# CPOMUCL/GPSat

Measured on AMD Instinct MI355X. Metric: local-expert tiles/sec (fit+predict), higher is better.
Workload: dtype f32; 1 GPU; BASELINE.json configs[1]: synthetic tiles, RBF, 3D inputs, fp32; tiles_per_gpu=4096, pred_per_tile=500, dim=3, kernel=RBF, optimiser=lbfgs, max_iter=20, early_stopping=ftol/gtol defaults, failed_tiles=0, parallelism=tile-sharded x1, device=AMD Radeon Graphics (gfx950:sramecc+:xnack-)

## Files before the change

gpsat_amd/csrc/gpsat_capi.cpp:

```cpp
#include <hip/hip_runtime.h>
#include <algorithm>
#include <cmath>
#include <cstdio>
#include <cstdlib>
#include <cstring>
#include <limits>
#include <numeric>
#include <string>
#include <vector>

#include "gpsat_hip.h"
#include "gpsat_kernels.h"
#include "gpsat_plan.h"
#include "gpsat_cvfold.h"
#include "gpsat_select_plan.h"
#include "gpsat_bin_plan.h"

namespace {

thread_local std::string g_err;

int fail(int code, const std::string& msg) {
    g_err = msg;
    return code;
// ... 435 lines not shown
    HIP_TRY(hipMemsetAsync(h->pq.p, 0, head, h->stream));
    char* q = static_cast<char*>(h->pq.p);
    a.pq_ctl = reinterpret_cast<int*>(q);
    a.cu_busy = reinterpret_cast<int*>(q + 256);
    a.pq = reinterpret_cast<unsigned long long*>(q + 256 + 2048 * sizeof(int));
    a.pq_snap = reinterpret_cast<float*>(q + head);
    a.pq_stride = p.pq_stride; a.pq_slots = (int)slots;
    return GPSAT_OK;
}

struct LaunchReport {
    std::vector<int> team, coop;
    int pq_taken = -1, unfinished = 0;
    bool team_gave_up = false;
};

int queue_report(gpsat_handle* h, const gpsat::TilePlan& p, const gpsat::KernelArgs& a, LaunchReport& r) {
    if (p.team > 1) {
        r.team.resize((size_t)(p.grid / p.team) * 64);
        HIP_TRY(hipMemcpyAsync(r.team.data(), h->coop.p, r.team.size() * sizeof(int), hipMemcpyDeviceToHost, h->stream));
    }
    if (p.coop && dev_env("GPSAT_DEBUG_COOP_STATS")) {
        r.coop.resize((size_t)p.grid * 256);
        HIP_TRY(hipMemcpyAsync(r.coop.data(), h->coop.p, (size_t)p.grid * 1024, hipMemcpyDeviceToHost, h->stream));
    }
    if (a.pq_ctl && dev_env("GPSAT_DEBUG_DEFER_STATS"))
        HIP_TRY(hipMemcpyAsync(&r.pq_taken, a.pq_ctl, sizeof(int), hipMemcpyDeviceToHost, h->stream));
    if (p.seg_cost > 0) HIP_TRY(hipMemcpyAsync(&r.unfinished, a.ring_ctl + 32, sizeof(int), hipMemcpyDeviceToHost, h->stream));
    return GPSAT_OK;
}

void read_report(const gpsat::TilePlan& p, const gpsat::KernelArgs& a, LaunchReport& r) {
    const int grid = p.grid, T = a.T;
    if (!r.coop.empty()) {
        long long st[8] = {0};
        for (int g = 0; g < grid; ++g) for (int i = 0; i < 8; ++i) st[i] += r.coop[(size_t)g * 256 + 32 + GPSAT_PT_MAXNB + i];
        std::fprintf(stderr, "gpsat coop: grid %d T %d: cooperative evaluations %lld, helper phases %lld, helper groups (sweep) %lld, "
                             "flag waits given up %lld, owner waits given up %lld, pivot failures %lld, helper unwinds %lld\n",
                     grid, T, st[0], st[1], st[2], st[3], st[4], st[5], st[6]);
    }
    if (dev_env("GPSAT_DEBUG_DEFER_STATS"))
        std::fprintf(stderr, "gpsat defer: T %d: deferred predictions %d of %d snapshot slots\n", T,
                     r.pq_taken < 0 ? 0 : std::min(r.pq_taken, a.pq_slots), a.pq_slots);
    if (!r.team.empty() && dev_env("GPSAT_DEBUG_TEAM_STATS"))
        std::fprintf(stderr, "gpsat team 0 (size %d), factorisation, owner thread 0, s_memtime ticks: own work of (A) %d, (A) wait + barrier %d, (B) + barrier %d, "
                             "(C) + barrier %d\n", p.team, r.team[24], r.team[25], r.team[26], r.team[27]);
    for (size_t g = 0; g < r.team.size() / 64; ++g)
        if (r.team[g * 64 + 5]) r.team_gave_up = true;
}

struct DenseJob {
    const gpsat_batch* b;
    const gpsat_multistart* ms;
    const gpsat_cv* cv = nullptr;
    CvTables cv_tables;
    bool ms_on;
    BatchDims dims;
    const double* theta0;
    std::vector<double> theta0_clipped, starts_clipped;
    std::vector<int> order;
};

int run_tiles(gpsat_handle* h, const DenseJob& j, bool solo, bool unsliced, LaunchReport& r) {
    const gpsat_batch* b = j.b;
    const BatchDims& d = j.dims;
    const bool f64 = b->dtype == GPSAT_F64;
    gpsat::PlanInput in = {b->T, b->D, f64, b->obs_off, d.maxP, d.want_cov, d.sumP > 0, b->optimiser, b->max_iter,
                           h->num_cu, h->wg_per_cu, solo || j.cv, unsliced, read_dev_knobs()};
    gpsat::TilePlan p;
    if (!gpsat::plan_tiles(in, p)) return fail(GPSAT_EINVAL, "tile too large for LDS");
    Staged s;
    int rc;
    const size_t ws_bytes = (size_t)(p.grid / p.team) * p.ws_stride * (f64 ? sizeof(double) : sizeof(float));
    if ((rc = stage_batch(h, b, d, j.theta0, j.order, d.want_cov ? b->cov_off : nullptr, nullptr, ws_bytes, s))) return rc;
    gpsat::KernelArgs a;
    fill_common_args(a, b, s);
    a.NBmax = p.NBmax;
    a.ws = static_cast<float*>(h->ws.p); a.ws_stride = p.ws_stride;
    a.prof = nullptr;
    a.cov_off = d.want_cov ? s.i64 + 2 * (b->T + 1) : nullptr;
    a.f_cov = d.want_cov ? reinterpret_cast<float*>(s.cov) : nullptr;
    a.PCmax = p.PCcov;
    a.dump = nullptr; a.dump_stride = 0;
    if ((rc = setup_ring(h, p, j.order, a))) return rc;
    if ((rc = setup_coop_and_team(h, p, &b->T, a))) return rc;
    if (j.ms_on && (rc = setup_multistart(h, b, j.ms->n_starts, j.theta0, j.starts_clipped, a))) return rc;
    if ((rc = setup_deferred(h, p, a))) return rc;
    gpsat::CvArgs ca;
    if (j.cv) {
        if (!gpsat::builds[p.build].launch_cv) return fail(GPSAT_EINVAL, "held-out predictions: no kernel in this build");
        if ((rc = stage_cv(h, b, j.cv, d, j.cv_tables, ca))) return rc;
    }
#ifdef GPSAT_DUMP
    if (h->dump_dev && !f64) {
        const size_t need = ((size_t)p.NBmax * p.NBmax + p.NBmax) * 1024 + 2 * (size_t)p.NBmax * 32 + 16 + 8 * 1024;
        if (h->dump_stride < need) return fail(GPSAT_EINVAL, "dump stride too small: need " + std::to_string(need) + " floats per tile");
        a.dump = h->dump_dev; a.dump_stride = h->dump_stride;
    }
#endif
#ifdef GPSAT_PROFILE
    if ((rc = h->prof.reserve(sizeof(h->prof_host)))) return rc;
    HIP_TRY(hipMemsetAsync(h->prof.p, 0, sizeof(h->prof_host), h->stream));
    a.prof = static_cast<unsigned long long*>(h->prof.p);
#endif
    HIP_TRY(hipEventRecord(h->ev[1], h->stream));
    if (j.cv) HIP_TRY(gpsat::builds[p.build].launch_cv(b->D, a, ca, p.grid, p.smem, h->stream));
    else HIP_TRY(gpsat::builds[p.build].launch(b->D, a, p.grid, p.smem, h->stream));
    HIP_TRY(hipEventRecord(h->ev[2], h->stream));
    if ((rc = fetch_batch(h, b, d, s))) return rc;
    if (j.cv && (rc = fetch_cv(h, b, j.cv, d, ca))) return rc;
    if (j.ms_on && j.ms->f_start)
        HIP_TRY(hipMemcpyAsync(j.ms->f_start, a.ms_fout, (size_t)b->T * j.ms->n_starts * sizeof(double), hipMemcpyDeviceToHost, h->stream));
#ifdef GPSAT_PROFILE
    HIP_TRY(hipMemcpyAsync(h->prof_host, h->prof.p, sizeof(h->prof_host), hipMemcpyDeviceToHost, h->stream));
#endif
    if ((rc = queue_report(h, p, a, r))) return rc;
    HIP_TRY(hipEventRecord(h->ev[3], h->stream));
    HIP_TRY(hipStreamSynchronize(h->stream));
    read_report(p, a, r);
    return GPSAT_OK;
}

int fit_predict(gpsat_handle* h, const gpsat_batch* b, const gpsat_multistart* ms, const gpsat_cv* cv = nullptr) {
    if (!h || !b) return fail(GPSAT_EINVAL, "gpsat_fit_predict_batch: NULL handle or batch");
    if (b->T == 0) return GPSAT_OK;
    DenseJob j;
    j.b = b; j.ms = ms; j.cv = cv;
    int rc;
    if ((rc = check_batch(b, false, j.dims))) return rc;
    BatchDims& d = j.dims;
    d.want_cov = b->f_cov != nullptr;
    if (d.want_cov) {
        if (!b->cov_off) return fail(GPSAT_EINVAL, "f_cov given without cov_off");
        if (b->cov_off[0] != 0) return fail(GPSAT_EINVAL, "cov_off must start at 0");
        for (int t = 0; t < b->T; ++t) {
            const long long p = b->pred_off[t + 1] - b->pred_off[t];
            if (b->cov_off[t + 1] - b->cov_off[t] != p * p) return fail(GPSAT_EINVAL, "cov_off[t+1]-cov_off[t] must equal P_t^2");
            d.maxP = std::max(d.maxP, p);
        }
        d.sumC = b->cov_off[b->T];
    }
    if (d.maxN > gpsat_max_tile_obs(b->dtype, b->D))
        return fail(GPSAT_EINVAL, "tile too large for the LDS of a CU: at most " + std::to_string(gpsat_max_tile_obs(b->dtype, b->D)) +
                                      " observations per tile for this dtype and D (gpsat_max_tile_obs)");
    if ((rc = check_batch_data(b, d))) return rc;
    if (cv && (rc = check_cv(b, cv, d, j.cv_tables))) return rc;
    j.ms_on = ms && b->optimiser != GPSAT_OPT_NONE && b->max_iter > 0;
    if (ms && (rc = check_multistart(b, ms, j.ms_on, j.theta0_clipped, j.starts_clipped))) return rc;
    j.theta0 = j.ms_on ? j.theta0_clipped.data() : b->theta0;
    if ((rc = begin_call(h))) return rc;
    j.order.resize(b->T);
    std::iota(j.order.begin(), j.order.end(), 0);
    std::stable_sort(j.order.begin(), j.order.end(), [&](int a, int c) {
        return (b->obs_off[a + 1] - b->obs_off[a]) > (b->obs_off[c + 1] - b->obs_off[c]);
    });
    for (bool solo = false, unsliced = false;;) {
        LaunchReport r;
        if ((rc = run_tiles(h, j, solo, unsliced, r))) return rc;
        if (r.team_gave_up) {
            std::fprintf(stderr, "gpsat: a team barrier gave up; re-running the batch with one workgroup per tile\n");
            solo = true;
        } else if (r.unfinished != 0) {
            if (unsliced) return fail(GPSAT_EHIP, "tile queue ended with " + std::to_string(r.unfinished) + " unfinished tiles");
            std::fprintf(stderr, "gpsat: time-sliced tile queue ended with %d unfinished tiles; re-running the batch unsliced\n", r.unfinished);
            unsliced = true;
        } else {
// ... 663 lines not shown
```

gpsat_amd/csrc/gpsat_kernels.h:

```cpp
#ifndef GPSAT_KERNELS_H
#define GPSAT_KERNELS_H
#include <hip/hip_runtime.h>
#include <stddef.h>

#include "gpsat_select_types.h"

#define GPSAT_MAX_TILE_OBS 4096
#define GPSAT_PT_MAXNB 128
static_assert(32 * GPSAT_PT_MAXNB >= GPSAT_MAX_TILE_OBS, "fp32 sweep flags must cover the largest tile gpsat_max_tile_obs allows");

namespace gpsat {

constexpr int MS_WORDS = 16;

struct KernelArgs {
    int T, kernel, optimiser, max_iter, max_ls, NBmax;
    double ftol, gtol, adam_lr;
    double noise_rel;
    const long long* obs_off;
    const long long* pred_off;
    const double* theta0;
    const double* lo;
    const double* hi;
    const unsigned char* trainable;
    const float* X;
    const float* y;
    const float* Xs;
    double* theta;
    double* nll;
    double* grad;
    int* status;
    int* n_eval;
    int* n_iter;
    float* f_mean;
    float* f_var;
    float* y_var;
    const int* order;
    int* queue;
    float* ws;
    size_t ws_stride;
    unsigned long long* prof;
    const long long* cov_off;
    float* f_cov;
    int PCmax;
    unsigned long long* ring;
    int* ring_ctl;
    unsigned* state;
    int ring_mask, state_words, seg_cost;
    void* coop;
    int* coop_live;
    int team_size;
    void* team_ctl;
    int coop_min_nb;
    int coop_hdiv;
    int coop_force;
    float* dump;
    size_t dump_stride;
    unsigned long long* pq;
    int* pq_ctl;
    int* cu_busy;
    float* pq_snap;
    size_t pq_stride;
    int pq_slots;
    int ms_S = 0;
    const double* ms_starts = nullptr;
    double* ms_state = nullptr;
    double* ms_fout = nullptr;
};

struct CvArgs {
    const int* pair_off = nullptr;
    const int* pairs = nullptr;
    const int* fold_off = nullptr;
    const int* fold_ptr = nullptr;
    const int* fold_rows = nullptr;
    const int* fold_a = nullptr;
    const int* row_fold = nullptr;
    const int* row_pos = nullptr;
    double* mean = nullptr;
    double* f_var = nullptr;
    double* y_var = nullptr;
};
#define GPSAT_MAX_CV_FOLD 256

size_t shared_bytes(int D, int NBmax);
size_t shared_bytes_f64(int D, int NBmax);
size_t workspace_doubles_per_wg_f64(int NBmax, int PCcov);
int state_words_f64();
hipError_t launch_tiles_f64(int D, const KernelArgs& a, int grid, size_t smem, hipStream_t stream);
hipError_t launch_tiles_cv_f64(int D, const KernelArgs& a, const CvArgs& cv, int grid, size_t smem, hipStream_t stream);
size_t shared_bytes_f64_w4(int D, int NBmax);
size_t workspace_doubles_per_wg_f64_w4(int NBmax, int PCcov);
int state_words_f64_w4();
hipError_t launch_tiles_f64_w4(int D, const KernelArgs& a, int grid, size_t smem, hipStream_t stream);
hipError_t launch_tiles_cv_f64_w4(int D, const KernelArgs& a, const CvArgs& cv, int grid, size_t smem, hipStream_t stream);
size_t pq_floats_per_slot(int D, int NBmax);
size_t workspace_floats_per_wg(int NBmax, int PCcov);
hipError_t launch_tiles(int D, const KernelArgs& a, int grid, size_t smem, hipStream_t stream);
int state_words();
size_t shared_bytes_w8(int D, int NBmax);
size_t workspace_floats_per_wg_w8(int NBmax, int PCcov);
hipError_t launch_tiles_w8(int D, const KernelArgs& a, int grid, size_t smem, hipStream_t stream);
int state_words_w8();

struct SelectArgs : SelectCriteria {
    long long M;
    int C;
    int T;
    const double* pts;
    const double* refs;
    int n_chunks;
    long long chunk_rows;
    long long* counts;
    const long long* off;
    int* idx;
    const double* box;
    const int* eorder;
    int n_bounds;
    const double* bounds;
};

hipError_t launch_select(const SelectArgs& a, bool fill, hipStream_t stream);
hipError_t launch_select_boxes(long long M, int C, const double* pts, double* box, hipStream_t stream);
int select_sub_rows();

hipError_t select_bin_rows(long long M, int C, const double* pts, const BinSpec& b, unsigned* keys, unsigned* keys_out, int* rows,
                           int* perm, double* pts_perm, void* temp, size_t& temp_bytes, hipStream_t stream);
hipError_t select_unbin(int T, long long total, const unsigned* seg_off, const int* perm, int* idx, int* idx_out, void* temp,
                        size_t& temp_bytes, hipStream_t stream);

#ifndef GPSAT_BIN_COUNT
#define GPSAT_BIN_COUNT  1u
#define GPSAT_BIN_SUM    2u
#define GPSAT_BIN_MEAN   4u
#define GPSAT_BIN_STD    8u
#define GPSAT_BIN_MIN    16u
#define GPSAT_BIN_MAX    32u
#define GPSAT_BIN_MEDIAN 64u
#endif
struct BinArgs {
    long long R;
    int nx, ny;
    const double *x, *y, *v;
    const int* gid;
    const double *ex, *ey;
    double x_hi, y_hi;
    double inv_x, inv_y;
    unsigned long long sentinel;
    unsigned long long *keys, *keys_sorted;
    unsigned *rows, *perm;
// ... 78 lines not shown
```

gpsat_amd/csrc/gpsat_kernels.hip:

```cpp
#include <hip/hip_runtime.h>
#include <stdint.h>
#include "gpsat_kernels.h"
#include "gpsat_ring.h"

#ifdef GPSAT_PROFILE
#define PROF_BEGIN() unsigned long long prof_t_ = __builtin_amdgcn_s_memtime()
#define PROF_END(c_, slot_)                                                                  \
    do {                                                                                     \
        unsigned long long t1_ = __builtin_amdgcn_s_memtime();                               \
        if ((c_).lane == 0) (c_).prof[(c_).w * 16 + (slot_)] += t1_ - prof_t_;               \
        prof_t_ = t1_;                                                                       \
    } while (0)
#define TRACE(c_, code_, arg_)                                                                        \
    do {                                                                                              \
        if ((c_).trace && (c_).lane == 0 && shared_state()->tron) {                                   \
            const int i_ = shared_state()->tcnt[(c_).w]++;                                            \
            if (i_ < 1024) (c_).trace[(c_).w * 1024 + i_] = (__builtin_amdgcn_s_memtime() << 16) |    \
                                                           ((unsigned long long)((arg_) & 255) << 8) | (code_); \
        }                                                                                             \
    } while (0)
#else
#define PROF_BEGIN() do {} while (0)
#define PROF_END(c_, slot_) do {} while (0)
#define TRACE(c_, code_, arg_) do {} while (0)
// ... 168 lines not shown
__device__ __forceinline__ void wave_lds_sync() {
    asm volatile("" ::: "memory");
    __builtin_amdgcn_wave_barrier();
    asm volatile("" ::: "memory");
}

__device__ __forceinline__ int wave_pull(int* counter, int lane) {
    int v = 0;
    if (lane == 0) v = atomicAdd(counter, 1);
    return __builtin_amdgcn_readfirstlane(v);
}

template <int KERN>
struct KScale {
    static constexpr float c = (KERN == 0) ? 0.8493218002880191f : 1.0f;
    static constexpr float c2 = (KERN == 0) ? 0.7213475204444817f : 1.0f;
};

template <int KERN>
__device__ __forceinline__ void kfun(float r2, float& kf, float& gg) {
    if (KERN == 0) {
        kf = __builtin_amdgcn_exp2f(-r2);
        gg = kf;
    } else {
        float r = sqrtf(fmaxf(r2, 1e-36f));
        if (KERN == 1) {
            kf = __expf(-r);
            gg = kf / r;
        } else if (KERN == 2) {
            float s = 1.7320508075688772f * r;
            float e = __expf(-s);
            kf = (1.f + s) * e;
            gg = 3.f * e;
        } else {
            float s = 2.23606797749979f * r;
            float e = __expf(-s);
            kf = (1.f + s + s * s * (1.f / 3.f)) * e;
            gg = (5.f / 3.f) * (1.f + s) * e;
        }
    }
}

#define GPSAT_PT_FLAGS
#include "gpsat_opt.h"
#include "gpsat_coop.h"

constexpr int SHARED_FLOATS = (int)((sizeof(Shared) + 15) / 16) * 4;

__device__ __forceinline__ Shared* shared_state() { return reinterpret_cast<Shared*>(lds_f); }

struct Lay { int xs, xsc, y, z, alpha, Ad, LT, U01, Wh, tmp, piv, end; };

__host__ __device__ constexpr Lay lds_layout(int D, int NBmax) {
    const int NPmax = NBmax * 32;
    Lay L{};
    int off = SHARED_FLOATS;
    L.xs = off; off += D * NPmax;
    L.xsc = off; off += D * NPmax;
    L.y = off; off += NPmax;
    L.z = off; off += NPmax;
    L.alpha = off; off += NPmax;
    L.LT = off; off += 4 * BLK;
    L.U01 = off; off += 2 * BLK;
    L.Wh = off; off += 4 * BLK;
    L.Ad = off; off += 32 * 33 + 3;
    off = (off + 3) & ~3;
    L.tmp = off; off += 32;
    L.piv = off; off += 64;
    L.end = off;
    return L;
}
constexpr int LDS_SLACK_FLOATS = 3;

template <int D, int KN>
struct Ctx {
    Lay L;
    float* ws;
    int zb, dT0, vs0, cv0;
    int gp0;
    gCoopCtl* ctl;
    gfloat* zg;
    gfloat* ag;
    bool helper;
    int N, NB, Npad, P;
    int tid, lane, w, h, g;
    float sf2, sn2;
    unsigned long long* prof;
    unsigned long long* trace;
};

template <int D, int KERN>
__device__ __forceinline__ f32x16 kblock_t(const Ctx<D, KERN>& c, int bi, int bj) {
    const int q = 32 * bj + c.g;
    float xq[D];
#pragma unroll
    for (int d = 0; d < D; ++d) xq[d] = lds_f[c.L.xsc + d * c.Npad + q];
    f32x16 out;
    if (bi != bj && 32 * bi + 32 <= c.N && 32 * bj + 32 <= c.N) {
#pragma unroll
        for (int qq = 0; qq < 4; ++qq) {
            const int p0 = 32 * bi + 8 * qq + 4 * c.h;
            f32x2 r2[2];
#pragma unroll
            for (int d = 0; d < D; ++d) {
                const f32x4 xp = *reinterpret_cast<const f32x4*>(lds_f + c.L.xsc + d * c.Npad + p0);
                const f32x2 xb = {xq[d], xq[d]};
#pragma unroll
                for (int e = 0; e < 2; ++e) {
                    const f32x2 xa = {xp[2 * e], xp[2 * e + 1]};
                    const f32x2 df = xa - xb;
                    r2[e] = (d == 0) ? df * df : __builtin_elementwise_fma(df, df, r2[e]);
                }
            }
#pragma unroll
            for (int e = 0; e < 4; ++e) {
                float kf, gg;
                kfun<KERN>(r2[e >> 1][e & 1], kf, gg);
                out[4 * qq + e] = c.sf2 * kf;
            }
        }
        return out;
    }
#pragma unroll
    for (int qq = 0; qq < 4; ++qq) {
        const int p0 = 32 * bi + 8 * qq + 4 * c.h;
        float r2[4] = {0.f, 0.f, 0.f, 0.f};
#pragma unroll
        for (int d = 0; d < D; ++d) {
            f32x4 xp = *reinterpret_cast<const f32x4*>(lds_f + c.L.xsc + d * c.Npad + p0);
#pragma unroll
            for (int e = 0; e < 4; ++e) { float df = xp[e] - xq[d]; r2[e] = fmaf(df, df, r2[e]); }
        }
#pragma unroll
        for (int e = 0; e < 4; ++e) {
            const int p = p0 + e;
            float kf, gg;
            kfun<KERN>(r2[e], kf, gg);
            float v = c.sf2 * kf;
            const bool valid = (p < c.N) && (q < c.N);
            v = valid ? v : 0.f;
            if (p == q) v = (p < c.N) ? (v + c.sn2) : 1.f;
            out[4 * qq + e] = v;
        }
    }
    return out;
}

template <int D, int KN>
__device__ __forceinline__ f32x16 kblock(const Ctx<D, KN>& c, int bi, int bj) {
    return kblock_t<D, KN>(c, bi, bj);
}

template <int D, int KERN>
__device__ __forceinline__ f32x16 ksblock_t(const Ctx<D, KERN>& c, int bj, const float (&xq)[D], bool qvalid) {
    f32x16 out;
#pragma unroll
    for (int qq = 0; qq < 4; ++qq) {
        const int p0 = 32 * bj + 8 * qq + 4 * c.h;
        float r2[4] = {0.f, 0.f, 0.f, 0.f};
#pragma unroll
        for (int d = 0; d < D; ++d) {
            f32x4 xp = *reinterpret_cast<const f32x4*>(lds_f + c.L.xsc + d * c.Npad + p0);
#pragma unroll
            for (int e = 0; e < 4; ++e) { float df = xp[e] - xq[d]; r2[e] = fmaf(df, df, r2[e]); }
        }
#pragma unroll
// ... 307 lines not shown
        __builtin_amdgcn_s_sleep(2);
        if (++spins > (1 << 22)) {
            __hip_atomic_store(&sh->fail, 2, __ATOMIC_RELAXED, __HIP_MEMORY_SCOPE_WORKGROUP);
            return false;
        }
    }
    __builtin_amdgcn_fence(__ATOMIC_ACQUIRE, "workgroup");
    return true;
}

__device__ __forceinline__ bool pt_wait_lc(Shared* sh, gCoopCtl* ctl, const int* flag, int v) {
    int spins = 0;
    while (__hip_atomic_load(flag, RLX_WG) < v) {
        if (__hip_atomic_load(&sh->fail, RLX_WG)) return false;
        __builtin_amdgcn_s_sleep(2);
        ++spins;
        if (((spins & 63) == 0 && __hip_atomic_load(&ctl->fail, RLX_AGENT)) || spins > (1 << 22)) {
            __hip_atomic_store(&sh->fail, 2, RLX_WG);
            return false;
        }
    }
    __builtin_amdgcn_fence(__ATOMIC_ACQUIRE, "workgroup");
    return true;
}

#define PTW(field, v) (COOP ? pt_wait_g(c.ctl, &c.ctl->field, (v)) : pt_wait(sh, &sh->field, (v)))
#define PTW_LOCAL(field, v) (COOP ? pt_wait_lc(sh, c.ctl, &sh->field, (v)) : pt_wait(sh, &sh->field, (v)))
#define PTS(field, v)                                                                     \
    do {                                                                                  \
        if (COOP) __hip_atomic_store(&c.ctl->field, (v), RLX_AGENT);                      \
        else __hip_atomic_store(&sh->field, (v), RLX_WG);                                 \
    } while (0)
#define PT_RELEASE() coop_drain()

#ifdef GPSAT_DUMP
#define DBG_TP(stage, jr, v) do { if ((jr) < 32) c.ws[(size_t)(c.zb - 8) * BLK + ((stage) * 32 + (jr)) * 64 + lane] = (v); } while (0)
#else
#define DBG_TP(stage, jr, v) do {} while (0)
#endif

template <int D, int KN>
__device__ __forceinline__ void chain_kloop(const Ctx<D, KN>& c, const Panel<D>& p, int kb, int ke, f32x16& D00, f32x16& D01,
                                            f32x16& D11, float& tp0, float& tp1) {
    const int NB = c.NB, lane = c.lane, j0 = p.j0, j1 = p.j1;
    const bool has1 = p.has1 != 0;
    if (kb >= ke) return;
    auto load = [&](RawHalf& a0, RawHalf& a1, int k, int m) {
        a0 = ldg_half(c.ws, k * NB + j0, m, lane);
        a1 = ldg_half(c.ws, has1 ? k * NB + j1 : c.zb, m, lane);
    };
    auto comp = [&](const RawHalf& a0, const RawHalf& a1, int k, int m) {
        HalfPl P0 = split_half(a0), P1 = split_half(a1);
        GPSAT_PLANES_SETTLE(GPSAT_PL(P0), GPSAT_PL(P1));
#define GPSAT_PP(i, j)                          \
        D00 = mfma_bf(P0.p[i], P0.p[j], D00);   \
        D01 = mfma_bf(P0.p[i], P1.p[j], D01);   \
        D11 = mfma_bf(P1.p[i], P1.p[j], D11);
        GPSAT_PP(1, 1) GPSAT_PP(0, 2) GPSAT_PP(2, 0) GPSAT_PP(0, 1) GPSAT_PP(1, 0) GPSAT_PP(0, 0)
#undef GPSAT_PP
#pragma unroll
        for (int q = 0; q < 8; ++q) {
            const float zk = lds_f[c.L.z + 32 * k + rho(8 * m + q, c.h)];
            tp0 = fmaf(__uint_as_float(a0.q[q >> 2][q & 3]), zk, tp0);
            tp1 = fmaf(__uint_as_float(a1.q[q >> 2][q & 3]), zk, tp1);
        }
    };
    const int n = 2 * (ke - kb);
    RawHalf a0[4], a1[4];
    auto load_i = [&](int slot, int i) { const int ii = max(min(i, n - 1), 0); load(a0[slot], a1[slot], kb + (ii >> 1), ii & 1); };
    load_i(0, 0); load_i(1, 1); load_i(2, 2);
    int i = 0;
    for (; i + 4 <= n; i += 4) {
#pragma unroll
        for (int u = 0; u < 4; ++u) {
            load_i((u + 3) & 3, i + u + 3);
            comp(a0[u], a1[u], kb + ((i + u) >> 1), (i + u) & 1);
        }
    }
#pragma unroll
    for (int u = 0; u < 3; ++u)
        if (i + u < n) comp(a0[u], a1[u], kb + ((i + u) >> 1), (i + u) & 1);
}

template <int D, int KN, bool COOP>
__device__ __forceinline__ bool pt_chain(Ctx<D, KN>& c, const Panel<D>& p, const Panel<D>& q, const bool want_m, int par,
                                         int kwait, int slot, bool held, int lt_users) {
    Shared* sh = shared_state();
    const int NB = c.NB, lane = c.lane;
    const int j0 = p.j0, j1 = p.j1;
    const bool has1 = p.has1 != 0;
    f32x16 D00 = zero16(), D01 = zero16(), D11 = zero16();
    float tp0 = 0.f, tp1 = 0.f;
    PROF_BEGIN();
    TRACE(c, 1, slot);
    if (slot >= 2) {
        if (!PTW(colrow[j0], slot - 1)) return false;
        if (has1 && !PTW(colrow[j1], slot - 1)) return false;
    }
    PROF_END(c, 10);
    __builtin_amdgcn_s_setprio(3);
    TRACE(c, 2, slot);
    chain_kloop<D, KN>(c, p, 0, kwait, D00, D01, D11, tp0, tp1);
    DBG_TP(0, j0, tp0); DBG_TP(0, j1, tp1);
    TRACE(c, 3, slot);
    if (kwait < j0 && !held) {
        PROF_END(c, 0);
        if (!PTW(g0done, slot)) { __builtin_amdgcn_s_setprio(0); return false; }
        PROF_END(c, 10);
        chain_kloop<D, KN>(c, p, kwait, j0, D00, D01, D11, tp0, tp1);
    }
    if (kwait < j0 && held) {
        PROF_END(c, 0);
        if (!PTW_LOCAL(parked, slot)) { __builtin_amdgcn_s_setprio(0); return false; }
        PROF_END(c, 10);
        TRACE(c, 4, slot);
        const int qpar = par ^ 1;
        const f32x16 L0 = ldl(c.L.LT + (2 * qpar + 0) * BLK, lane);
        const f32x16 L1 = ldl(c.L.LT + (2 * qpar + 1) * BLK, lane);
        const f32x16 Uq = ldl(c.L.U01 + qpar * BLK, lane);
        f32x16 X0[2], X1[2];
        f32x16 Wp[4];
#pragma unroll
        for (int n = 0; n < 4; ++n) Wp[n] = ldl(c.L.Wh + n * BLK, lane);
        wave_lds_sync();
        if (lane == 0) __hip_atomic_store(&sh->whfree, slot, __ATOMIC_RELAXED, __HIP_MEMORY_SCOPE_WORKGROUP);
#pragma unroll
        for (int n = 0; n < 2; ++n) {
            const f32x16 W0 = Wp[n];
            f32x16 W1 = Wp[2 + n];
            X0[n] = zero16();
            mma_blk(X0[n], L0, W0);
            f32x16 T = zero16();
            mma_blk(T, Uq, X0[n]);
            W1 -= T;
            X1[n] = zero16();
            mma_blk(X1[n], L1, W1);
            stg(c.ws, q.j0 * NB + j0 + n, lane, X0[n]);
            stg(c.ws, q.j1 * NB + j0 + n, lane, X1[n]);
        }
        mma_blk(D00, X0[0], X0[0]); mma_blk(D00, X1[0], X1[0]);
        mma_blk(D01, X0[0], X0[1]); mma_blk(D01, X1[0], X1[1]);
        mma_blk(D11, X0[1], X0[1]); mma_blk(D11, X1[1], X1[1]);
#pragma unroll
        for (int qq = 0; qq < 16; ++qq) {
            const float z0 = lds_f[c.L.z + 32 * q.j0 + rho(qq, c.h)], z1 = lds_f[c.L.z + 32 * q.j1 + rho(qq, c.h)];
            tp0 = fmaf(X0[0][qq], z0, fmaf(X1[0][qq], z1, tp0));
            tp1 = fmaf(X0[1][qq], z0, fmaf(X1[1][qq], z1, tp1));
        }
        PT_RELEASE();
        if (lane == 0) PTS(g0done, slot);
    }
    PROF_END(c, 0);
    DBG_TP(1, j0, tp0); DBG_TP(1, j1, tp1);
    TRACE(c, 5, slot);
    if (slot >= 2 && !COOP) {
        if (!pt_wait(sh, &sh->gdone[par], lt_users)) { __builtin_amdgcn_s_setprio(0); return false; }
        if (lane == 0) __hip_atomic_store(&sh->gdone[par], 0, __ATOMIC_RELAXED, __HIP_MEMORY_SCOPE_WORKGROUP);
        PROF_END(c, 10);
    }
    TRACE(c, 6, slot);
    f32x16 S1keep = zero16();
    const int nrow = has1 ? 2 : 1;
    for (int r = 0; r < nrow; ++r) {
        const int jr = j0 + r;
        f32x16 Dd;
        float tp;
        if (r == 0) {
            Dd = kblock<D, KN>(c, j0, j0) - D00;
            tp = tp0;
        } else {
            const f32x16 U01 = ldl(c.L.U01 + par * BLK, lane);
            mma_blk(D11, U01, U01);
#pragma unroll
            for (int q = 0; q < 16; ++q) tp1 = fmaf(U01[q], lds_f[c.L.z + 32 * j0 + rho(q, c.h)], tp1);
            Dd = kblock<D, KN>(c, j1, j1) - D11;
            tp = tp1;
        }
        f32x16 S1, S2;
        double ls;
        int bad;
        PROF_END(c, 2);
        diag_factor(Dd, c.L.Ad, c.L.piv, lane, S1, S2, ls, bad);
        PROF_END(c, 1);
        TRACE(c, 7 + r, slot);
        stg(c.ws, jr * NB + jr, lane, S1);
// ... 55 lines not shown
        }
    }
    __builtin_amdgcn_s_setprio(0);
    PT_RELEASE();
    if (lane == 0) {
        PTS(colrow[j0], slot + 1);
        if (has1) PTS(colrow[j1], slot + 1);
        PTS(ready, slot + 1);
    }
    PROF_END(c, 2);
    TRACE(c, 9, slot);
    return true;
}

template <int D>
__device__ __forceinline__ Panel<D> make_panel(int NB, int pi, bool want_m) {
    Panel<D> p;
    p.j0 = 2 * pi;
    p.j1 = p.j0 + 1;
    p.has1 = (p.j1 < NB) ? 1 : 0;
    p.nU = p.has1 ? (NB - 1 - p.j1) : 0;
    p.nItems = p.nU + (want_m ? p.j0 : 0);
    return p;
}

template <int D>
__device__ __forceinline__ int pt_lt_users(const Panel<D>& q) { return ((q.nItems + 1) >> 1) - (q.nU >= 2 ? 1 : 0); }

template <int D, int KN, bool COOP>
__device__ __forceinline__ bool pt_run_group(const Ctx<D, KN>& c, const Panel<D>& q, int sq, int g, bool queued) {
    Shared* sh = shared_state();
    PROF_BEGIN();
    TRACE(c, 20, sq * 16 + g);
#pragma unroll
    for (int n = 0; n < 2; ++n) {
        const int e = 2 * g + n;
        if (e < q.nItems && !PTW(colrow[pt_item_col(q, e)], sq)) return false;
    }
    if (sq >= 1 && !PTW(g0done, sq)) return false;
    PROF_END(c, 3);
    TRACE(c, 21, sq * 16 + g);
    f32x16 W[4];
    pt_group_kloop<D, KN>(c, q, g, W);
    PROF_END(c, 4);
    TRACE(c, 22, sq * 16 + g);
    if (!PTW(ready, sq + 1)) return false;
    if (COOP && c.helper && 2 * g + 1 >= q.nU) {
        const int i = 32 * q.j0 + c.lane;
        if (i < c.Npad) lds_f[c.L.z + i] = gld_f(c.zg + i);
        wave_lds_sync();
    }
    PROF_END(c, 3);
    TRACE(c, 24, sq * 16 + g);
    float apsum[2] = {0.f, 0.f};
    pt_group_row<D, KN, COOP>(c, q, g, 0, sq & 1, W, apsum);
    if (q.has1) pt_group_row<D, KN, COOP>(c, q, g, 1, sq & 1, W, apsum);
    PT_RELEASE();
    if (c.lane == 0) {
#pragma unroll
        for (int n = 0; n < 2; ++n) {
            const int e = 2 * g + n;
            if (e < q.nItems) PTS(colrow[pt_item_col(q, e)], sq + 1);
        }
        if (COOP) { if (queued) __hip_atomic_fetch_add(&c.ctl->done, 1, RLX_AGENT); if (c.helper) COOP_STAT(c.ctl, 2); }
        else __hip_atomic_fetch_add(&sh->gdone[sq & 1], 1, RLX_WG);
    }
    PROF_END(c, 5);
    TRACE(c, 23, sq * 16 + g);
    return true;
}

template <int D>
__device__ __forceinline__ int pt_queue_len(int NB, bool want_m) {
    const int NP = (NB + 1) >> 1;
    int tot = 0;
    for (int s = 0; s < NP; ++s) {
        const Panel<D> q = make_panel<D>(NB, s, want_m);
        tot += max(0, ((q.nItems + 1) >> 1) - ((s == NP - 1) ? 0 : 2));
    }
    return tot;
}

template <int D, int KN, bool COOP>
__device__ __forceinline__ bool pt_bulk_loop(const Ctx<D, KN>& c, const bool want_m, bool ok) {
    Shared* sh = shared_state();
    const int NB = c.NB;
    const int NP = (NB + 1) >> 1;
    int sq = 0, base = 0;
    Panel<D> q = make_panel<D>(NB, 0, want_m);
    int g0 = (NP == 1) ? 0 : 2;
    int nq = max(0, ((q.nItems + 1) >> 1) - g0);
    while (ok) {
        int idx;
        if (COOP) {
            int v = 0;
            if (c.lane == 0) v = __hip_atomic_fetch_add(&c.ctl->qhead, 1, RLX_AGENT);
            idx = __builtin_amdgcn_readfirstlane(v);
        } else {
            idx = wave_pull(&sh->qhead, c.lane);
        }
        while (sq < NP && idx >= base + nq) {
            base += nq;
            ++sq;
            if (sq < NP) {
                q = make_panel<D>(NB, sq, want_m);
                g0 = (sq == NP - 1) ? 0 : 2;
                nq = max(0, ((q.nItems + 1) >> 1) - g0);
            }
        }
        if (sq >= NP) break;
        TRACE(c, 50, sq);
        ok = pt_run_group<D, KN, COOP>(c, q, sq, g0 + idx - base, true);
    }
    return ok;
}

__device__ __forceinline__ bool coop_wait_eq(gCoopCtl* ctl, const gint* word, int v) {
    for (int spins = 0; __hip_atomic_load(word, RLX_AGENT) != v; ++spins) {
        __builtin_amdgcn_s_sleep(8);
        if (spins > (1 << 21)) { COOP_STAT(ctl, 4); return false; }
        if ((spins & 15) == 15 && __hip_atomic_load(&ctl->fail, RLX_AGENT)) return false;
    }
    return true;
}

__device__ __forceinline__ void coop_open(Shared* sh, gCoopCtl* ctl, int kind) {
    sh->coop_seq += 1;
    __hip_atomic_store(&ctl->pa, PA_MAKE(sh->coop_seq, kind), RLX_AGENT);
}

__device__ __forceinline__ bool coop_close(Shared* sh, gCoopCtl* ctl, int total) {
    bool ok = coop_wait_eq(ctl, &ctl->done, total);
    __hip_atomic_fetch_and(&ctl->pa, ~(3ull << 32), RLX_AGENT);
    for (int spins = 0; PA_ACTIVE(__hip_atomic_load(&ctl->pa, RLX_AGENT)) != 0u; ++spins) {
        __builtin_amdgcn_s_sleep(8);
        if (spins > (1 << 21)) { COOP_STAT(ctl, 4); ok = false; break; }
    }
    return ok;
}

template <int D, int KN, bool COOP>
__device__ __forceinline__ void phase_pt(Ctx<D, KN>& c, const bool want_m) {
    Shared* sh = shared_state();
    const int NB = c.NB, w = c.w;
    const int NP = (NB + 1) >> 1;
    if (c.tid == 0) {
        sh->logdet = 0.0; sh->fail = 0; sh->g0done = 0; sh->ready = 0; sh->parked = 0; sh->whfree = 0;
        sh->gdone[0] = 0; sh->gdone[1] = 0; sh->qhead = 0;
    }
    for (int idx = c.tid; idx < NB; idx += NT) sh->colrow[idx] = 0;
    for (int idx = c.tid; idx < c.Npad; idx += NT) lds_f[c.L.alpha + idx] = 0.f;
    if (COOP) {
        if (c.tid == 0) {
            __hip_atomic_store(&c.ctl->ready, 0, RLX_AGENT);
            __hip_atomic_store(&c.ctl->g0done, 0, RLX_AGENT);
            __hip_atomic_exchange(&c.ctl->qhead, 0, RLX_AGENT);
            __hip_atomic_exchange(&c.ctl->done, 0, RLX_AGENT);
            __hip_atomic_exchange(&c.ctl->fail, 0, RLX_AGENT);
            __hip_atomic_store(&c.ctl->want_m, want_m ? 1 : 0, RLX_AGENT);
        }
        for (int idx = c.tid; idx < NB; idx += NT) __hip_atomic_store(&c.ctl->colrow[idx], 0, RLX_AGENT);
        for (int idx = c.tid; idx < c.Npad; idx += NT) gst_f(c.ag + idx, 0.f);
        coop_drain();
        __syncthreads();
        if (c.tid == 0) { coop_open(sh, c.ctl, COOP_SWEEP); COOP_STAT(c.ctl, 0); }
    }
    __syncthreads();
    bool ok = true;
    if (w == 0) {
        for (int s = 0; s < NP && ok; ++s) {
            const Panel<D> p = make_panel<D>(NB, s, want_m);
            const Panel<D> q = make_panel<D>(NB, s > 0 ? s - 1 : 0, want_m);
            const int kwait = (s > 0) ? (p.j0 - 2) : p.j0;
            const bool held = (s > 0) && (q.nU >= 2);
            const int users = (s >= 2) ? pt_lt_users<D>(make_panel<D>(NB, s - 2, want_m)) : 0;
            ok = pt_chain<D, KN, COOP>(c, p, q, want_m, s & 1, kwait, s, held, users);
            if (ok && __hip_atomic_load(&sh->fail, RLX_WG)) ok = false;
        }
    } else if (w == 1) {
        for (int s = 0; s < NP && ok; ++s) {
            if (s >= 1) {
                const Panel<D> q = make_panel<D>(NB, s - 1, want_m);
                const int nGroups = (q.nItems + 1) >> 1;
                if (ok && nGroups > 0 && q.nU < 2) {
                    ok = pt_run_group<D, KN, COOP>(c, q, s - 1, 0, false);
                    if (ok && c.lane == 0) PTS(g0done, s);
                }
                if (NW < 8 && ok && nGroups > 1) ok = pt_run_group<D, KN, COOP>(c, q, s - 1, 1, false);
            }
            if (ok && s < NP) {
                const Panel<D> pn = make_panel<D>(NB, s, want_m);
                if (pn.nU >= 2) {
                    PROF_BEGIN();
                    ok = PTW(colrow[pn.j1 + 1], s) && PTW(colrow[pn.j1 + 2], s);
                    if (ok && s >= 1) ok = PTW(g0done, s);
                    if (ok) ok = PTW_LOCAL(whfree, s);
                    PROF_END(c, 3);
                    TRACE(c, 30, s);
                    if (ok) {
                        f32x16 W[4];
                        pt_group_kloop<D, KN>(c, pn, 0, W);
#pragma unroll
                        for (int n = 0; n < 4; ++n) stl(c.L.Wh + n * BLK, c.lane, W[n]);
                        wave_lds_sync();
                        if (c.lane == 0) __hip_atomic_store(&sh->parked, s + 1, RLX_WG);
                        PROF_END(c, 4);
                        TRACE(c, 31, s);
                    }
                }
            }
        }
    }
    if (NW >= 8 && w == 2) {
        for (int s = 1; s < NP && ok; ++s) {
            const Panel<D> q = make_panel<D>(NB, s - 1, want_m);
            if (((q.nItems + 1) >> 1) > 1) ok = pt_run_group<D, KN, COOP>(c, q, s - 1, 1, false);
        }
    }
    ok = pt_bulk_loop<D, KN, COOP>(c, want_m, ok);
    if (COOP && !ok && c.lane == 0) {
        __hip_atomic_store(&sh->fail, 2, RLX_WG);
        __hip_atomic_store(&c.ctl->fail, 2, RLX_AGENT);
    }
    TRACE(c, 60, 0);
    coop_drain();
    __syncthreads();
    if (COOP) {
        if (c.tid == 0) {
            if (!coop_close(sh, c.ctl, pt_queue_len<D>(NB, want_m)) && !sh->fail) sh->fail = 2;
            if (__hip_atomic_load(&c.ctl->fail, RLX_AGENT) && !sh->fail) sh->fail = 2;
        }
// ... 515 lines not shown
__device__ __forceinline__ int pq_block(int b, int NB) {
    const int nu = NB * (NB - 1) / 2;
    if (b >= nu) return NB * NB + (b - nu);
    int j = 1;
    while ((j + 1) * j / 2 <= b) ++j;
    return (b - j * (j - 1) / 2) * NB + j;
}

template <int D, int KN>
__device__ void pq_save(Ctx<D, KN>& c, const KernelArgs& A, int s, int t, const float (&invl)[D]) {
    const int NB = c.NB, nblk = NB * (NB - 1) / 2 + NB;
    float* snap = A.pq_snap + (size_t)s * A.pq_stride;
    for (int b = c.w; b < nblk; b += NW) stg(snap, b, c.lane, ldg(c.ws, pq_block(b, NB), c.lane));
    unsigned* tail = reinterpret_cast<unsigned*>(snap + (size_t)nblk * BLK);
    for (int i = c.tid; i < (D + 1) * c.Npad; i += NT) {
        const float v = i < c.Npad ? lds_f[c.L.z + i] : lds_f[c.L.xsc + i - c.Npad];
        __hip_atomic_store(&tail[i], __float_as_uint(v), __ATOMIC_RELAXED, __HIP_MEMORY_SCOPE_AGENT);
    }
    if (c.tid == 0) {
        unsigned* hdr = tail + (D + 1) * c.Npad;
        __hip_atomic_store(&hdr[0], __float_as_uint(c.sf2), __ATOMIC_RELAXED, __HIP_MEMORY_SCOPE_AGENT);
        __hip_atomic_store(&hdr[1], __float_as_uint(c.sn2), __ATOMIC_RELAXED, __HIP_MEMORY_SCOPE_AGENT);
#pragma unroll
        for (int d = 0; d < D; ++d) __hip_atomic_store(&hdr[2 + d], __float_as_uint(invl[d]), __ATOMIC_RELAXED, __HIP_MEMORY_SCOPE_AGENT);
    }
    asm volatile("s_waitcnt vmcnt(0)" ::: "memory");
    __syncthreads();
    if (c.tid == 0) pq_publish(A, s, t);
}

template <int D, int KN>
__device__ void pq_predict(Ctx<D, KN>& c, const KernelArgs& A, int s, int t, float* ws_own) {
    const long long o0 = A.obs_off[t], o1 = A.obs_off[t + 1];
    const long long p0 = A.pred_off[t], p1 = A.pred_off[t + 1];
    c.N = (int)(o1 - o0);
    c.P = (int)(p1 - p0);
    c.NB = (c.N + 31) / 32;
    c.Npad = c.NB * 32;
    const int NB = c.NB, nblk = NB * (NB - 1) / 2 + NB;
    c.dT0 = NB * NB;
    c.vs0 = c.dT0 + NB;
    c.cv0 = c.vs0 + NW * 2 * NB;
    c.ws = ws_own;
    const float* snap = A.pq_snap + (size_t)s * A.pq_stride;
    for (int b = c.w; b < nblk; b += NW) stg(c.ws, pq_block(b, NB), c.lane, ldg(snap, b, c.lane));
    const unsigned* tail = reinterpret_cast<const unsigned*>(snap + (size_t)nblk * BLK);
    for (int i = c.tid; i < (D + 1) * c.Npad; i += NT) {
        const float v = __uint_as_float(__hip_atomic_load(&tail[i], __ATOMIC_RELAXED, __HIP_MEMORY_SCOPE_AGENT));
        if (i < c.Npad) lds_f[c.L.z + i] = v; else lds_f[c.L.xsc + i - c.Npad] = v;
    }
    c.sf2 = __uint_as_float(__hip_atomic_load(&tail[(D + 1) * c.Npad], __ATOMIC_RELAXED, __HIP_MEMORY_SCOPE_AGENT));
    c.sn2 = __uint_as_float(__hip_atomic_load(&tail[(D + 1) * c.Npad + 1], __ATOMIC_RELAXED, __HIP_MEMORY_SCOPE_AGENT));
    float invl[D];
#pragma unroll
    for (int d = 0; d < D; ++d)
        invl[d] = __uint_as_float(__hip_atomic_load(&tail[(D + 1) * c.Npad + 2 + d], __ATOMIC_RELAXED, __HIP_MEMORY_SCOPE_AGENT));
    asm volatile("s_waitcnt vmcnt(0)" ::: "memory");
    __syncthreads();
    predict_tile<D, KN>(c, A.Xs + (size_t)p0 * D, A.f_mean + p0, A.f_var + p0, A.y_var + p0, invl, nullptr);
    asm volatile("s_waitcnt vmcnt(0)" ::: "memory");
    __syncthreads();
    if (c.tid == 0) __hip_atomic_fetch_add(&A.ring_ctl[32], -1, __ATOMIC_RELAXED, __HIP_MEMORY_SCOPE_AGENT);
}

template <int D, int KN>
__global__ void __launch_bounds__(NT, GPSAT_MIN_WG) gp_tile_kernel(const KernelArgs A) {
    constexpr int H = D + 2;
    Ctx<D, KN> c;
    c.tid = threadIdx.x;
    c.lane = c.tid & 63;
    c.w = c.tid >> 6;
    c.h = c.lane >> 5;
    c.g = c.lane & 31;
    Shared* sh = shared_state();
    c.L = lds_layout(D, A.NBmax);
    float* const ws_own = A.ws + (size_t)blockIdx.x * A.ws_stride;
    c.ws = ws_own;
    c.zb = (int)(A.ws_stride / BLK) - 1;
    if (c.w == 0) { stg(c.ws, c.zb, c.lane, zero16()); coop_drain(); }
    constexpr bool COOP_BUILD = (NW == 8);
    const bool coop_on = COOP_BUILD && A.coop != nullptr;
    gCoopCtl* const ctl_own = as_gctl(A.coop) + blockIdx.x;
    if (c.tid == 0) { sh->hp[0] = -1; sh->hp[1] = -1; sh->hp[2] = -1; sh->coop_now = 0; sh->coop_seq = 0; }
    c.prof = sh->prof;
    c.trace = nullptr;
#ifdef GPSAT_PROFILE
    if (blockIdx.x == 0 && A.prof) c.trace = A.prof + 64;
    if (c.tid < NW) sh->tcnt[c.tid] = 0;
    int prof_ntiles = 0;
    unsigned long long prof_empty = 0;
    if (c.tid < NW * 16) sh->prof[c.tid] = 0ull;
    const unsigned long long prof_k0 = __builtin_amdgcn_s_memtime(), prof_r0 = __builtin_amdgcn_s_memrealtime();
#endif
    OptCfg o = opt_cfg(A);
    o.ms_S = A.ms_S; o.ms_starts = A.ms_starts; o.ms_state = A.ms_state; o.ms_fout = A.ms_fout;

    const bool sliced = A.seg_cost > 0;
    const bool defer_on = (NW == 4) && sliced && A.pq != nullptr;
    const int my_cu = defer_on ? cu_index() : 0;
#ifdef GPSAT_PROFILE
    unsigned long long prof_pred = 0;
#endif
    for (;;) {
        __syncthreads();
        HelpArgs ha;
        ha.coop = A.coop; ha.ws = A.ws; ha.ws_stride = A.ws_stride; ha.obs_off = A.obs_off; ha.X = A.X;
        ha.grid = (int)gridDim.x;
        ha.xcd_mode = (A.coop_force >> 2) & 3;
        if (sliced && coop_on) {
            if (c.tid == 0) sh->hp[7] = (int)ring_claim(A);
            for (int spins = 0;; ++spins) {
                if (c.tid == 0) sh->tile = (spins > (1 << 22)) ? -1 : ring_look(A, (unsigned)sh->hp[7]);
                __syncthreads();
                if (sh->tile != -2) break;
                helper_episode<D, KN>(c, ha);
            }
        } else if (defer_on) {
#ifdef GPSAT_PROFILE
            const unsigned long long tw0 = __builtin_amdgcn_s_memtime();
            if (c.tid == 0 && prof_empty == 0 && ring_waiting_tiles(A) <= 0) prof_empty = __builtin_amdgcn_s_memrealtime();
            prof_pred = 0;
#endif
            if (c.tid == 0) sh->hp[7] = (int)ring_claim(A);
            for (int spins = 0;;) {
                if (c.tid == 0) {
                    int e = ring_look(A, (unsigned)sh->hp[7]);
                    sh->hp[5] = -1;
                    if (e == -2) {
                        if (spins > (1 << 25)) e = -1;
                        else {
                            const int q = __hip_atomic_load(&A.cu_busy[my_cu], __ATOMIC_RELAXED, __HIP_MEMORY_SCOPE_AGENT) == 0 ? pq_claim(A) : -1;
                            if (q >= 0) { sh->hp[5] = q; sh->hp[4] = pq_wait_entry(A, q); }
                            else { ++spins; __builtin_amdgcn_s_sleep(64); }
                        }
                    }
                    sh->tile = e;
                }
                __syncthreads();
                const int e = sh->tile, q = sh->hp[5], qt = sh->hp[4];
                __syncthreads();
                if (e != -2) break;
                if (q >= 0 && qt >= 0) {
#ifdef GPSAT_PROFILE
                    const unsigned long long tp0 = __builtin_amdgcn_s_memtime();
#endif
                    pq_predict<D, KN>(c, A, q, qt, ws_own);
#ifdef GPSAT_PROFILE
                    prof_pred += __builtin_amdgcn_s_memtime() - tp0;
#endif
                }
            }
#ifdef GPSAT_PROFILE
            if (c.tid == 0) sh->prof[13] += __builtin_amdgcn_s_memtime() - tw0 - prof_pred;
#endif
        } else if (c.tid == 0) {
            if (sliced) {
#ifdef GPSAT_PROFILE
                const unsigned long long tw0 = __builtin_amdgcn_s_memtime();
                if (prof_empty == 0 && ring_waiting_tiles(A) <= 0) prof_empty = __builtin_amdgcn_s_memrealtime();
#endif
                sh->tile = ring_pop(A);
#ifdef GPSAT_PROFILE
                sh->prof[13] += __builtin_amdgcn_s_memtime() - tw0;
#endif
            } else {
                const int slot = atomicAdd(A.queue, 1);
                sh->tile = slot < A.T ? A.order[slot] : -1;
            }
        }
        __syncthreads();
        int entry = sh->tile;
        if (entry == -1 && coop_on && !sliced) {
            for (;;) {
                if (c.tid == 0) sh->hp[6] = __hip_atomic_load(A.coop_live, RLX_AGENT);
                __syncthreads();
                if (sh->hp[6] <= 0) break;
                helper_episode<D, KN>(c, ha);
            }
        }
        if (entry == -1) break;
#ifdef GPSAT_PROFILE
        if (c.tid == 0) sh->tron = (prof_ntiles == 2);
// ... 223 lines not shown
```

gpsat_amd/csrc/gpsat_opt.h:

```cpp
#ifndef GPSAT_OPT_H
#define GPSAT_OPT_H

#ifndef GPSAT_NW
#define GPSAT_NW 4
#endif
constexpr int NW = GPSAT_NW;
constexpr int NT = 64 * NW;
constexpr int HMAX = 6;
constexpr int MH = 10;

struct Shared {
    double theta[HMAX];
    double gth[HMAX];
    double nll;
    double logdet;
    double red[8][8];
    double lo[HMAX], hi[HMAX], shift[HMAX];
    double u[HMAX], g[HMAX], f;
    double ut[HMAX], gt[HMAX], ft;
    double ub[HMAX], gb[HMAX];
    double d[HMAX];
    double S[MH][HMAX], Y[MH][HMAX], rho_[MH];
    double m1[HMAX], m2[HMAX];
    double t, t_prev, f_prev, dphi_prev, t_lo, f_lo, dphi_lo, t_hi, f_hi, dphi_hi, dphi0, t_best, f_best, last_dec;
    int ls_phase, ls_iter, ls_done, ls_ok;
    int hist_n, hist_pos;
    int trainable[HMAX];
    int box[HMAX];
    int fail, done, status, n_eval, n_eval_opt, iter, phase, want_grad;
    int tile;
    int g0done;
    int gnext[2];
#ifdef GPSAT_PT_FLAGS
    int ready, parked, whfree;
    int gdone[2];
    int qhead;
    int colrow[GPSAT_PT_MAXNB];
#endif
    int gradnext;
    int coop_seq;
    int coop_now;
    int hp[8];
#ifdef GPSAT_PROFILE
    unsigned long long prof[NW * 16];
    int tcnt[NW], tron;
#else
    unsigned long long prof[1];
#endif
};


static __device__ inline double softplus_d(double x) { return log1p(exp(-fabs(x))) + fmax(x, 0.0); }

static __device__ __noinline__ double theta_of_u(const Shared* sh, int i, double u) {
    if (sh->box[i] == 2) return exp(u);
    if (sh->box[i]) return sh->lo[i] + (sh->hi[i] - sh->lo[i]) / (1.0 + exp(-u));
    return softplus_d(u) + sh->shift[i];
}

static __device__ __noinline__ double u_of_theta(const Shared* sh, int i, double th) {
    if (sh->box[i] == 2) return log(th);
    if (sh->box[i]) {
        const double lo = sh->lo[i], hi = sh->hi[i];
        double t = (th - lo) / (hi - lo);
        t = fmin(fmax(t, 1e-15), 1.0 - 1e-15);
        return log(t / (1.0 - t));
    }
    double y = th - sh->shift[i];
    if (y < 1e-300) y = 1e-300;
    if (y > 34.0) return y;
    if (y < 1e-15) return log(y);
    return log(-expm1(-y)) + y;
}

static __device__ inline double dtheta_du(const Shared* sh, int i, double th) {
    if (sh->box[i] == 2) return th;
    if (sh->box[i]) return (th - sh->lo[i]) * (sh->hi[i] - th) / (sh->hi[i] - sh->lo[i]);
    return -expm1(-(th - sh->shift[i]));
}

static __device__ __noinline__ void set_trial(Shared* sh, int H, const double* u) {
    for (int i = 0; i < H; ++i) {
        sh->ut[i] = u[i];
        if (sh->trainable[i]) sh->theta[i] = theta_of_u(sh, i, u[i]);
    }
}

static __device__ __noinline__ void fetch_trial(Shared* sh, int H) {
    sh->ft = sh->fail ? __builtin_inf() : sh->nll;
    for (int i = 0; i < H; ++i)
        sh->gt[i] = (sh->trainable[i] && !sh->fail) ? sh->gth[i] * dtheta_du(sh, i, sh->theta[i]) : 0.0;
}

static __device__ __noinline__ void lbfgs_direction(Shared* sh, int H) {
    double q[HMAX], al[MH];
    for (int i = 0; i < H; ++i) q[i] = sh->g[i];
    const int n = sh->hist_n;
    for (int m = 0; m < n; ++m) {
        const int idx = (sh->hist_pos - 1 - m + 2 * MH) % MH;
        double a = 0.0;
        for (int i = 0; i < H; ++i) a += sh->S[idx][i] * q[i];
        a *= sh->rho_[idx];
        al[m] = a;
        for (int i = 0; i < H; ++i) q[i] -= a * sh->Y[idx][i];
    }
    if (n > 0) {
        const int idx = (sh->hist_pos - 1 + MH) % MH;
        double sy = 0.0, yy = 0.0;
        for (int i = 0; i < H; ++i) { sy += sh->S[idx][i] * sh->Y[idx][i]; yy += sh->Y[idx][i] * sh->Y[idx][i]; }
        const double gam = sy / yy;
        for (int i = 0; i < H; ++i) q[i] *= gam;
    }
    for (int m = n - 1; m >= 0; --m) {
        const int idx = (sh->hist_pos - 1 - m + 2 * MH) % MH;
        double b = 0.0;
        for (int i = 0; i < H; ++i) b += sh->Y[idx][i] * q[i];
        b *= sh->rho_[idx];
        for (int i = 0; i < H; ++i) q[i] += (al[m] - b) * sh->S[idx][i];
    }
    for (int i = 0; i < H; ++i) sh->d[i] = -q[i];
// ... 583 lines not shown
```

Before: 33700 tiles/s.

## Precompute next diagonal panel chain ahead in idle bulk-loop waves

Adds a look-ahead path: while waves loop over bulk Cholesky panel work, one wave may claim the next diagonal panel, run its k-loop update early, and park the partial results in workspace. The chain step then loads the parked values instead of recomputing them when another wave already claimed that slot. This is meant to shorten the serial critical path of the panel-by-panel factorisation. It adds workgroup atomics, extra global stores and loads, and a possible early return when parked data is not ready yet. It is on by default with rule 1, and an env var can change it.

```diff
diff --git a/gpsat_amd/csrc/gpsat_capi.cpp b/gpsat_amd/csrc/gpsat_capi.cpp
--- a/gpsat_amd/csrc/gpsat_capi.cpp
+++ b/gpsat_amd/csrc/gpsat_capi.cpp
@@ -541,6 +541,7 @@
     a.f_cov = d.want_cov ? reinterpret_cast<float*>(s.cov) : nullptr;
     a.PCmax = p.PCcov;
     a.dump = nullptr; a.dump_stride = 0;
+    if (const char* e = dev_env("GPSAT_DEBUG_DIAG_AHEAD")) a.diag_ahead = std::atoi(e);
     if ((rc = setup_ring(h, p, j.order, a))) return rc;
     if ((rc = setup_coop_and_team(h, p, &b->T, a))) return rc;
     if (j.ms_on && (rc = setup_multistart(h, b, j.ms->n_starts, j.theta0, j.starts_clipped, a))) return rc;
diff --git a/gpsat_amd/csrc/gpsat_kernels.h b/gpsat_amd/csrc/gpsat_kernels.h
--- a/gpsat_amd/csrc/gpsat_kernels.h
+++ b/gpsat_amd/csrc/gpsat_kernels.h
@@ -66,6 +66,7 @@
     const double* ms_starts = nullptr;
     double* ms_state = nullptr;
     double* ms_fout = nullptr;
+    int diag_ahead = 1;
 };
 
 struct CvArgs {
diff --git a/gpsat_amd/csrc/gpsat_kernels.hip b/gpsat_amd/csrc/gpsat_kernels.hip
--- a/gpsat_amd/csrc/gpsat_kernels.hip
+++ b/gpsat_amd/csrc/gpsat_kernels.hip
@@ -274,6 +274,8 @@
     gfloat* zg;
     gfloat* ag;
     bool helper;
+    int drule;
+    const int* dbusy;
     int N, NB, Npad, P;
     int tid, lane, w, h, g;
     float sf2, sn2;
@@ -747,6 +749,40 @@
         if (i + u < n) comp(a0[u], a1[u], kb + ((i + u) >> 1), (i + u) & 1);
 }
 
+__device__ __forceinline__ bool pt_diag_claim(Shared* sh, int from, int to, int lane) {
+    int won = 0;
+    if (lane == 0) {
+        int expect = from;
+        won = __hip_atomic_compare_exchange_strong(&sh->dclaim, &expect, to, __ATOMIC_RELAXED, __ATOMIC_RELAXED,
+                                                   __HIP_MEMORY_SCOPE_WORKGROUP) ? 1 : 0;
+    }
+    return __builtin_amdgcn_readfirstlane(won) != 0;
+}
+
+template <int D, int KN>
+__device__ __forceinline__ void pt_diag_park(const Ctx<D, KN>& c, int par, const f32x16& D00, const f32x16& D01, const f32x16& D11,
+                                             float tp0, float tp1) {
+    const int b = c.vs0 + 4 * par;
+    stg(c.ws, b, c.lane, D00);
+    stg(c.ws, b + 1, c.lane, D01);
+    stg(c.ws, b + 2, c.lane, D11);
+    gfloat* t = as_gfloat(c.ws + (size_t)(b + 3) * BLK);
+    gst_f(t + c.lane, tp0);
+    gst_f(t + 64 + c.lane, tp1);
+}
+
+template <int D, int KN>
+__device__ __forceinline__ void pt_diag_load(const Ctx<D, KN>& c, int par, f32x16& D00, f32x16& D01, f32x16& D11, float& tp0,
+                                             float& tp1) {
+    const int b = c.vs0 + 4 * par;
+    D00 = ldg(c.ws, b, c.lane);
+    D01 = ldg(c.ws, b + 1, c.lane);
+    D11 = ldg(c.ws, b + 2, c.lane);
+    const gfloat* t = as_gfloat(c.ws + (size_t)(b + 3) * BLK);
+    tp0 = gld_f(t + c.lane);
+    tp1 = gld_f(t + 64 + c.lane);
+}
+
 template <int D, int KN, bool COOP>
 __device__ __forceinline__ bool pt_chain(Ctx<D, KN>& c, const Panel<D>& p, const Panel<D>& q, const bool want_m, int par,
                                          int kwait, int slot, bool held, int lt_users) {
@@ -765,7 +801,14 @@
     PROF_END(c, 10);
     __builtin_amdgcn_s_setprio(3);
     TRACE(c, 2, slot);
-    chain_kloop<D, KN>(c, p, 0, kwait, D00, D01, D11, tp0, tp1);
+    if (slot < 2 || !c.drule || pt_diag_claim(sh, slot - 1, slot, lane)) {
+        chain_kloop<D, KN>(c, p, 0, kwait, D00, D01, D11, tp0, tp1);
+    } else {
+        PROF_END(c, 0);
+        if (!PTW_LOCAL(dparked[par], slot)) { __builtin_amdgcn_s_setprio(0); return false; }
+        PROF_END(c, 10);
+        pt_diag_load<D, KN>(c, par, D00, D01, D11, tp0, tp1);
+    }
     DBG_TP(0, j0, tp0); DBG_TP(0, j1, tp1);
     TRACE(c, 3, slot);
     if (kwait < j0 && !held) {
@@ -987,6 +1030,48 @@
 }
 
 template <int D, int KN, bool COOP>
+__device__ __forceinline__ void pt_diag_ahead(const Ctx<D, KN>& c, const bool want_m) {
+    Shared* sh = shared_state();
+    const int NP = (c.NB + 1) >> 1;
+    const int d = __builtin_amdgcn_readfirstlane(__hip_atomic_load(&sh->dclaim, RLX_WG));
+    const int s = d + 1;
+    if (s >= NP) return;
+    const Panel<D> p = make_panel<D>(c.NB, s, want_m);
+    int r0, r1;
+    if (COOP) {
+        r0 = __hip_atomic_load(&c.ctl->colrow[p.j0], RLX_AGENT);
+        r1 = p.has1 ? __hip_atomic_load(&c.ctl->colrow[p.j1], RLX_AGENT) : s;
+    } else {
+        r0 = __hip_atomic_load(&sh->colrow[p.j0], RLX_WG);
+        r1 = p.has1 ? __hip_atomic_load(&sh->colrow[p.j1], RLX_WG) : s;
+    }
+    if (__builtin_amdgcn_readfirstlane(min(r0, r1)) < s - 1) return;
+    if (c.drule & 2) {
+        const int rd = COOP ? __hip_atomic_load(&c.ctl->ready, RLX_AGENT) : __hip_atomic_load(&sh->ready, RLX_WG);
+        if (__builtin_amdgcn_readfirstlane(rd) >= s) return;
+    }
+    if (c.drule & 4) {
+        if (!c.dbusy) return;
+        if (__builtin_amdgcn_readfirstlane(__hip_atomic_load(c.dbusy, RLX_AGENT)) > 1) return;
+    }
+    if (!pt_diag_claim(sh, d, s, c.lane)) return;
+    __builtin_amdgcn_fence(__ATOMIC_ACQUIRE, "workgroup");
+    PROF_BEGIN();
+    TRACE(c, 40, s);
+    f32x16 D00 = zero16(), D01 = zero16(), D11 = zero16();
+    float tp0 = 0.f, tp1 = 0.f;
+    chain_kloop<D, KN>(c, p, 0, p.j0 - 2, D00, D01, D11, tp0, tp1);
+    pt_diag_park<D, KN>(c, s & 1, D00, D01, D11, tp0, tp1);
+    PT_RELEASE();
+    if (c.lane == 0) __hip_atomic_store(&sh->dparked[s & 1], s, RLX_WG);
+    PROF_END(c, 11);
+#ifdef GPSAT_PROFILE
+    if (c.lane == 0) c.prof[c.w * 16 + 13] += 1;
+#endif
+    TRACE(c, 41, s);
+}
+
+template <int D, int KN, bool COOP>
 __device__ __forceinline__ bool pt_bulk_loop(const Ctx<D, KN>& c, const bool want_m, bool ok) {
     Shared* sh = shared_state();
     const int NB = c.NB;
@@ -996,6 +1081,7 @@
     int g0 = (NP == 1) ? 0 : 2;
     int nq = max(0, ((q.nItems + 1) >> 1) - g0);
     while (ok) {
+        if (c.drule && !(COOP && c.helper)) pt_diag_ahead<D, KN, COOP>(c, want_m);
         int idx;
         if (COOP) {
             int v = 0;
@@ -1052,6 +1138,7 @@
     if (c.tid == 0) {
         sh->logdet = 0.0; sh->fail = 0; sh->g0done = 0; sh->ready = 0; sh->parked = 0; sh->whfree = 0;
         sh->gdone[0] = 0; sh->gdone[1] = 0; sh->qhead = 0;
+        sh->dclaim = 1; sh->dparked[0] = 0; sh->dparked[1] = 0;
     }
     for (int idx = c.tid; idx < NB; idx += NT) sh->colrow[idx] = 0;
     for (int idx = c.tid; idx < c.Npad; idx += NT) lds_f[c.L.alpha + idx] = 0.f;
@@ -1733,6 +1820,8 @@
     const bool coop_on = COOP_BUILD && A.coop != nullptr;
     gCoopCtl* const ctl_own = as_gctl(A.coop) + blockIdx.x;
     if (c.tid == 0) { sh->hp[0] = -1; sh->hp[1] = -1; sh->hp[2] = -1; sh->coop_now = 0; sh->coop_seq = 0; }
+    c.drule = A.diag_ahead;
+    c.dbusy = nullptr;
     c.prof = sh->prof;
     c.trace = nullptr;
 #ifdef GPSAT_PROFILE
@@ -1749,6 +1838,7 @@
     const bool sliced = A.seg_cost > 0;
     const bool defer_on = (NW == 4) && sliced && A.pq != nullptr;
     const int my_cu = defer_on ? cu_index() : 0;
+    if (defer_on) c.dbusy = A.cu_busy + my_cu;
 #ifdef GPSAT_PROFILE
     unsigned long long prof_pred = 0;
 #endif
diff --git a/gpsat_amd/csrc/gpsat_opt.h b/gpsat_amd/csrc/gpsat_opt.h
--- a/gpsat_amd/csrc/gpsat_opt.h
+++ b/gpsat_amd/csrc/gpsat_opt.h
@@ -36,6 +36,8 @@
     int gdone[2];
     int qhead;
     int colrow[GPSAT_PT_MAXNB];
+    int dclaim;
+    int dparked[2];
 #endif
     int gradnext;
     int coop_seq;
```

New measurement: 33160 tiles/s. 0.984x the previous value.
